# real-stanford/semantic-abstraction

Hardware: AMD Instinct MI355X
Metric: scenes/sec (relevancy+3D-UNet infer), 480x480x16-label x128^3 (higher is better)
Workload: dtype f16 (MFMA operands, fp32 accumulate; UNet hi/lo-split = fp32-equivalent); 1 GPU; end-to-end relevancy->fusion->OVSSC per scene: 480x480 RGB-D, 16 labels, ViT-B/16, 'ours' saliency config (2448 tile forwards), 128^3 voxels, 80000 input points; scene-sharded; arch=ViT-B/16, unet_precision=exact, tile_chunk_streams=1, scenes_per_gpu=26, parallelism=scene-shard x1, mode=throughput

## Files before the change

### semantic-abstraction_amd/csrc/unet.hip

```cpp
#include "semabs_common.h"

__device__ __forceinline__ int xcd_remap(int vb, int nb) {
    const int q = nb >> 3, r = nb & 7, x = vb & 7, k = vb >> 3;
    return (x < r ? x * (q + 1) : r * (q + 1) + (x - r) * q) + k;
}
__device__ __forceinline__ int xcd_persistent_tile(int vb, int G, int it, int total) {
    if (G & 7) { const long t = (long)it * G + vb; return t < total ? (int)t : -1; }
    const int x = vb & 7, j = vb >> 3, g8 = G >> 3;
    const int q = total >> 3, r = total & 7;
    const int lo = x < r ? x * (q + 1) : r * (q + 1) + (x - r) * q, cnt = q + (x < r ? 1 : 0);
    const long o = (long)it * g8 + j;
    return o < cnt ? lo + (int)o : -1;
}


template <int HID, int COUT>
__global__ __launch_bounds__(256, 2) void k_point_mlp(const float* __restrict__ xyz, const float* __restrict__ feat,
                                                   const float* __restrict__ w1, const float* __restrict__ b1,
                                                   const float* __restrict__ w2, const float* __restrict__ b2,
                                                   const float* __restrict__ w3, const float* __restrict__ b3,
                                                   float* __restrict__ out, int P, long N) {
    extern __shared__ __attribute__((aligned(16))) char smem[];
    float* sw2 = reinterpret_cast<float*>(smem);
    float* sw3 = sw2 + HID * HID;
// ... 374 lines not shown
    SEMABS_REQUIRE(sums && gamma && beta && scale && shift && C % G == 0 && nvox > 0, "semabs_gn_finalize: bad args");
    hipLaunchKernelGGL(k_gn_finalize, dim3(semabs_cdiv((long)B * C, 256)), dim3(256), 0, (hipStream_t)stream, sums, gamma, beta, scale,
                       shift, B, C, G, (double)nvox * (C / G), eps);
    SEMABS_CHECK_LAUNCH();
    return SEMABS_OK;
}

#ifdef SEMABS_TUNING
#define CONV16_ABL(c) (c)
#else
#define CONV16_ABL(c) false
#endif
struct ConvArgs {
    const void* x; void* y; const f16* w_hi; const f16* w_lo;
    const float* gn_scale; const float* gn_shift; const float* bias; const void* resid;
    int B, I0, I1, I2;
    int O0, O1, O2;
    int M0, M1, M2;
    int os, op0, op1, op2;
    int Cin, Cout, Kp;
    int ntaps; int relu;
    int is;
    int ksplit;
    signed char td0[28], td1[28], td2[28];
    double* stats;
    int ablate;
    long long* trace;
    const f16* wp_hi; const f16* wp_lo;
    int ncls; long cls_off[8];
    const float* gnb_coef = nullptr; const float* gnb_mean = nullptr; const float* gnb_rstd = nullptr; int gnb_G = 0, gnb_relu = 0;
    unsigned int* gnb_bits = nullptr;
    const unsigned int* occ = nullptr;
    const float* gnb_add = nullptr;
};

template <bool F32>
__device__ __forceinline__ void load8(const void* base, long idx, float (&v)[8]) {
    if (F32) {
        const float4* p = reinterpret_cast<const float4*>(reinterpret_cast<const float*>(base) + idx);
        float4 a = p[0], b = p[1];
        v[0] = a.x; v[1] = a.y; v[2] = a.z; v[3] = a.w; v[4] = b.x; v[5] = b.y; v[6] = b.z; v[7] = b.w;
    } else {
        f16x8 h = *reinterpret_cast<const f16x8*>(reinterpret_cast<const f16*>(base) + idx);
#pragma unroll
        for (int j = 0; j < 8; ++j) v[j] = (float)h[j];
    }
}

template <int NW, bool F32, bool CIN16, bool LDSW = false, bool CLS = false>
__global__ __launch_bounds__(256) void k_conv(ConvArgs a) {
    const int ccls = CLS ? (int)blockIdx.z : 0;
    const int cp0 = CLS ? ccls >> 2 : 0, cp1 = CLS ? (ccls >> 1) & 1 : 0, cp2 = CLS ? ccls & 1 : 0;
    const int k_ntaps = CLS ? (cp0 + 1) * (cp1 + 1) * (cp2 + 1) : a.ntaps;
    const int k_Kp = CLS ? k_ntaps * a.Cin : a.Kp;
    const int k_op0 = CLS ? cp0 : a.op0, k_op1 = CLS ? cp1 : a.op1, k_op2 = CLS ? cp2 : a.op2;
    const long k_woff = CLS ? a.cls_off[ccls] : 0;
    const f16* const k_w_hi = a.w_hi + k_woff; const f16* const k_w_lo = a.w_lo ? a.w_lo + k_woff : nullptr;
    const f16* const k_wp_hi = a.wp_hi ? a.wp_hi + k_woff : nullptr; const f16* const k_wp_lo = a.wp_lo ? a.wp_lo + k_woff : nullptr;
    constexpr int MW = 2;
    static_assert(!LDSW || (NW == 4 && !CIN16), "LDSW: four waves x four output-channel tiles");
    __shared__ __attribute__((aligned(16))) f16x8 s_w[LDSW ? 2 : 1][LDSW ? 4 : 1][2][LDSW ? 64 : 1];
    const int lane = threadIdx.x & 63, wid = threadIdx.x >> 6;
    const int vl = lane & 15, kg = lane >> 4;
    const long Mtot = (long)a.B * a.M0 * a.M1 * a.M2;
    const long mbase = ((long)blockIdx.x * 4 + wid) * (MW * 16);
    if (!LDSW && mbase >= Mtot) return;
// ... 456 lines not shown
                for (int j = 0; j < 4; ++j) st[j] += (double)ps[j];
            }
        }
    };

    auto lds_barrier = [&]() { asm volatile("s_waitcnt lgkmcnt(0)\n\ts_barrier" ::: "memory"); };
    auto brick_of = [&](int it) { return xcd_persistent_tile((int)blockIdx.x, (int)gridDim.x, it, total); };
    if (producer) {
        int it = 0, brick = brick_of(0);
        if (brick >= 0) produce(brick, 0);
        lds_barrier();
        int buf = 0;
        for (; brick >= 0; buf ^= 1) {
            const int next = brick_of(++it);
            if (next >= 0 && !CONV16_ABL(a.ablate == 2 || a.ablate >= 4)) produce(next, buf ^ 1);
            lds_barrier();
            brick = next;
        }
    } else {
        load_weights();
        lds_barrier();
        int buf = 0, it = 0;
        for (int brick = brick_of(0); brick >= 0; brick = brick_of(++it), buf ^= 1) {
            if (!CONV16_ABL(a.ablate == 1)) consume(brick, buf);
            lds_barrier();
        }
        if (a.stats) flush_stats();
        if (GNB && a.gnb_bits) conv_absmax_commit(a.gnb_bits, amax);
    }
}

#define SEMABS_CONV_GENERIC 256
#define SEMABS_CONV_PACKED 512
#ifdef SEMABS_TUNING
static int g_conv16_ablate = 0;
static long long* g_conv_trace = nullptr;
static int g_brick_persist = 0;
static int g_convt_no_line = 0;
extern "C" int semabs_conv_tune(int key, long long value) {
    if (key == 0) g_conv16_ablate = (int)value & 7;
    else if (key == 1) g_conv_trace = reinterpret_cast<long long*>(value);
    else if (key == 2) g_brick_persist = (int)value;
    else if (key == 3) g_convt_no_line = (int)value;
    return SEMABS_OK;
}
#endif

static int conv16_lds_launch(const ConvArgs& a_in, int f32, hipStream_t s) {
    ConvArgs a = a_in;
#ifdef SEMABS_TUNING
    a.ablate = g_conv16_ablate;
#endif
    if (f32) {
        constexpr int T0 = 4;
        const size_t lds = (size_t)(((T0 + 2) * C16_H1 * C16_H2 * 8 + 127) / 128 * 128) * 2 * 2 * 2 * 2;
        const long total = (long)a.B * (a.I0 / T0) * (a.I1 / C16_T1) * (a.I2 / C16_T2);
        long nb = semabs_stream_cus(s); if (nb > total) nb = total;
        if (a.gnb_coef) {
            static SemabsLdsAttr attrg;
            semabs_ensure_lds(&k_conv16_lds<true, T0, true>, (int)(lds + 32 * 192), attrg);
            hipLaunchKernelGGL((k_conv16_lds<true, T0, true>), dim3((unsigned)nb), dim3(512), lds + (size_t)a.B * 192, s, a);
            SEMABS_CHECK_LAUNCH();
            return SEMABS_OK;
        }
        if (a.occ) {
            static SemabsLdsAttr attrs;
            semabs_ensure_lds(&k_conv16_lds<true, T0, false, true>, (int)lds, attrs);
            hipLaunchKernelGGL((k_conv16_lds<true, T0, false, true>), dim3((unsigned)nb), dim3(512), lds, s, a);
            SEMABS_CHECK_LAUNCH();
            return SEMABS_OK;
        }
        static SemabsLdsAttr attr;
        semabs_ensure_lds(&k_conv16_lds<true, T0>, (int)lds, attr);
        hipLaunchKernelGGL((k_conv16_lds<true, T0>), dim3((unsigned)nb), dim3(512), lds, s, a);
    } else {
        constexpr int T0 = 8;
// ... 349 lines not shown
    }
    BRICK_STAMP(7);
}

template <bool F32, int CW, int NB, bool ONE, bool PERSIST, int TX = 16, bool GNB = false>
static int conv_brick_launch_p(const ConvArgs& a, hipStream_t s) {
    const size_t lds = (size_t)((6 * C16_H1 * (TX + 2) * 8 + 127) / 128 * 128) * (CW / 8) * 2 * (F32 ? 2 : 1);
    static int per_cu = 0;
    if (!per_cu) {
        (void)hipFuncSetAttribute(reinterpret_cast<const void*>(&k_conv_brick<F32, CW, NB, ONE, PERSIST, TX, GNB>), hipFuncAttributeMaxDynamicSharedMemorySize, (int)lds);
        int n = 0;
        if (hipOccupancyMaxActiveBlocksPerMultiprocessor(&n, k_conv_brick<F32, CW, NB, ONE, PERSIST, TX, GNB>, 512, lds) != hipSuccess || n < 1) n = 1;
        per_cu = n;
    }
    const long total = (long)(a.I0 / 4) * (a.I1 / C16_T1) * (a.I2 / TX) * a.B * (a.Cout / (NB * 16));
    SEMABS_REQUIRE(total < (1L << 30), "conv brick: too many tiles");
    long nwg = total;
    if (PERSIST) { nwg = (long)semabs_stream_cus(s) * per_cu; if (nwg > total) nwg = total; }
    ConvArgs at = a;
#ifdef SEMABS_TUNING
    at.trace = g_conv_trace;
#endif
    hipLaunchKernelGGL((k_conv_brick<F32, CW, NB, ONE, PERSIST, TX, GNB>), dim3((unsigned)nwg), dim3(512), lds, s, at, (int)total);
    SEMABS_CHECK_LAUNCH();
    return SEMABS_OK;
}
template <bool F32, int CW, int NB, bool ONE>
static int conv_brick_launch_t(const ConvArgs& a, hipStream_t s) {
#ifdef SEMABS_TUNING
    if (g_brick_persist) return conv_brick_launch_p<F32, CW, NB, ONE, true>(a, s);
#endif
    return conv_brick_launch_p<F32, CW, NB, ONE, false>(a, s);
}
static int conv_brick_launch(const ConvArgs& a, int f32, hipStream_t s) {
    if (a.gnb_coef) {
        if (a.Cin == 32) return conv_brick_launch_p<true, 32, 2, true, false, 16, true>(a, s);
        return conv_brick_launch_p<true, 32, 2, false, false, 16, true>(a, s);
    }
    if (a.I2 % C16_T2 != 0) {
        return f32 ? conv_brick_launch_p<true, 32, 2, false, false, 8>(a, s) : conv_brick_launch_p<false, 32, 2, false, false, 8>(a, s);
    }
    const long bricks = (long)a.B * (a.I0 / 4) * (a.I1 / C16_T1) * (a.I2 / C16_T2);
    if (a.Cout == 16) {
        if (a.Cin == 32) return f32 ? conv_brick_launch_t<true, 32, 1, true>(a, s) : conv_brick_launch_t<false, 32, 1, true>(a, s);
        return f32 ? conv_brick_launch_t<true, 32, 1, false>(a, s) : conv_brick_launch_t<false, 32, 1, false>(a, s);
    }
    const bool nb4 = a.Cout % 64 == 0 && bricks * (a.Cout / 64) >= 512;
    if (a.Cin == 16) {
        if (nb4) return f32 ? conv_brick_launch_t<true, 16, 4, true>(a, s) : conv_brick_launch_t<false, 16, 4, true>(a, s);
        return f32 ? conv_brick_launch_t<true, 16, 2, true>(a, s) : conv_brick_launch_t<false, 16, 2, true>(a, s);
    }
    if (a.Cin == 32) {
        if (nb4) return f32 ? conv_brick_launch_t<true, 32, 4, true>(a, s) : conv_brick_launch_t<false, 32, 4, true>(a, s);
        return f32 ? conv_brick_launch_t<true, 32, 2, true>(a, s) : conv_brick_launch_t<false, 32, 2, true>(a, s);
    }
    if (nb4) return f32 ? conv_brick_launch_t<true, 32, 4, false>(a, s) : conv_brick_launch_t<false, 32, 4, false>(a, s);
    return f32 ? conv_brick_launch_t<true, 32, 2, false>(a, s) : conv_brick_launch_t<false, 32, 2, false>(a, s);
}

__global__ void k_conv_finish(float* __restrict__ y, const float* __restrict__ bias, const float* __restrict__ resid, long n4, int C, int relu) {
    const long i = (long)blockIdx.x * blockDim.x + threadIdx.x;
    if (i >= n4) return;
    float4 v = *reinterpret_cast<float4*>(y + i * 4);
    if (bias) { const float4 b = *reinterpret_cast<const float4*>(bias + (i * 4) % C); v.x += b.x; v.y += b.y; v.z += b.z; v.w += b.w; }
    if (resid) { const float4 r = *reinterpret_cast<const float4*>(resid + i * 4); v.x += r.x; v.y += r.y; v.z += r.z; v.w += r.w; }
    if (relu == 1) { v.x = fmaxf(v.x, 0.f); v.y = fmaxf(v.y, 0.f); v.z = fmaxf(v.z, 0.f); v.w = fmaxf(v.w, 0.f); }
    else if (relu == 2) { v.x = v.x > 0.f ? v.x : 0.01f * v.x; v.y = v.y > 0.f ? v.y : 0.01f * v.y; v.z = v.z > 0.f ? v.z : 0.01f * v.z; v.w = v.w > 0.f ? v.w : 0.01f * v.w; }
    *reinterpret_cast<float4*>(y + i * 4) = v;
}

static int conv_launch(const ConvArgs& a_in, int f32, hipStream_t s) {
    ConvArgs a = a_in;
    const long Mtot = (long)a.B * a.M0 * a.M1 * a.M2;
    a.ksplit = 1;
    if (f32 && a.os == 1 && a.Cout % 64 == 0 && a.Cin % 32 == 0 && a.ntaps == 27 && Mtot <= 16384) {
        const long slices = semabs_cdiv(Mtot, 4 * 32) * (a.Cout / 64);
        int ks = (int)(2048 / (slices > 0 ? slices : 1));
        if (ks > 27) ks = 27;
        if (ks >= 3) {
// ... 5 lines not shown
            hipLaunchKernelGGL(k_conv_finish, dim3(semabs_cdiv(n4, 256)), dim3(256), 0, s, reinterpret_cast<float*>(a.y), a.bias,
                               reinterpret_cast<const float*>(a.resid), n4, a.Cout, a.relu);
            SEMABS_CHECK_LAUNCH();
            return SEMABS_OK;
        }
    }
    const int ncls = a.ncls > 0 ? a.ncls : 1;
    int nw = a.Cout >= 64 ? 4 : (a.Cout >= 32 ? 2 : 1);
    while (nw > 1 && (long)semabs_cdiv(Mtot, 4 * 32) * (a.Cout / (nw * 16)) * ncls < 1024) nw >>= 1;
    dim3 grid(semabs_cdiv(Mtot, 4 * 32), a.Cout / (nw * 16), ncls), block(256);
    const bool c16 = a.Cin == 16;
    if (a.ncls > 0) {
#define CONVC_GO(NW_, F_) hipLaunchKernelGGL((k_conv<NW_, F_, false, false, true>), grid, block, 0, s, a)
        if (f32) { if (nw == 4) CONVC_GO(4, true); else if (nw == 2) CONVC_GO(2, true); else CONVC_GO(1, true); }
        else { if (nw == 4) CONVC_GO(4, false); else if (nw == 2) CONVC_GO(2, false); else CONVC_GO(1, false); }
#undef CONVC_GO
        SEMABS_CHECK_LAUNCH();
        return SEMABS_OK;
    }
#define CONV_GO(NW_, F_, C_) hipLaunchKernelGGL((k_conv<NW_, F_, C_>), grid, block, 0, s, a)
#define CONV_NW(F_, C_) { if (nw == 4) CONV_GO(4, F_, C_); else if (nw == 2) CONV_GO(2, F_, C_); else CONV_GO(1, F_, C_); }
    if (nw == 4 && !c16) {
        if (f32) hipLaunchKernelGGL((k_conv<4, true, false, true>), grid, block, 0, s, a);
        else hipLaunchKernelGGL((k_conv<4, false, false, true>), grid, block, 0, s, a);
    }
    else if (f32) { if (c16) CONV_NW(true, true) else CONV_NW(true, false) }
    else { if (c16) CONV_NW(false, true) else CONV_NW(false, false) }
#undef CONV_NW
#undef CONV_GO
    SEMABS_CHECK_LAUNCH();
    return SEMABS_OK;
}

static int conv_common_checks(const void* x, const void* w_hi, const void* w_lo, void* y, int Cin, int Cout, int f32) {
    SEMABS_REQUIRE(x && w_hi && y, "semabs conv: null pointer");
    SEMABS_REQUIRE(!f32 || w_lo, "semabs conv: exact (fp32) mode needs the lo half of the split weights");
    SEMABS_REQUIRE(Cin == 16 || Cin % 32 == 0, "semabs conv: Cin must be 16 or a multiple of 32");
    SEMABS_REQUIRE(Cout % 16 == 0 && (Cout < 64 || Cout % 64 == 0), "semabs conv: Cout must be 16, 32 or a multiple of 64");
    return SEMABS_OK;
}

static int conv3d_impl(const void* x, const void* w_hi, const void* w_lo, void* y, const float* gn_scale, const float* gn_shift,
                       const float* bias, const void* resid, int B, int D0, int D1, int D2, int Cin, int Cout, int ksize,
                       int relu, int act_flags, double* out_sums, int out_groups, void* stream, const unsigned int* occ = nullptr) {
    if (B == 0) return SEMABS_OK;
    const int act_f32 = act_flags & 1;
    const bool bricks = !(act_flags & SEMABS_CONV_GENERIC);
    int rc = conv_common_checks(x, w_hi, w_lo, y, Cin, Cout, act_f32);
    if (rc) return rc;
    SEMABS_REQUIRE(ksize == 1 || ksize == 3, "semabs_conv3d: kernel size must be 1 or 3");
    SEMABS_REQUIRE((gn_scale == nullptr) == (gn_shift == nullptr), "semabs_conv3d: gn_scale and gn_shift go together");
    ConvArgs a;
    a.x = x; a.y = y; a.w_hi = (const f16*)w_hi; a.w_lo = (const f16*)w_lo; a.gn_scale = gn_scale; a.gn_shift = gn_shift;
    a.bias = bias; a.resid = resid; a.B = B; a.I0 = D0; a.I1 = D1; a.I2 = D2; a.O0 = D0; a.O1 = D1; a.O2 = D2;
    a.M0 = D0; a.M1 = D1; a.M2 = D2; a.os = 1; a.is = 1; a.op0 = a.op1 = a.op2 = 0; a.Cin = Cin; a.Cout = Cout; a.relu = relu;
    a.ntaps = ksize * ksize * ksize;
    a.Kp = ((a.ntaps * Cin + 31) / 32) * 32;
    a.stats = nullptr; a.ablate = 0; a.trace = nullptr; a.wp_hi = nullptr; a.wp_lo = nullptr; a.ncls = 0;
    if (act_flags & SEMABS_CONV_PACKED) {
        a.wp_hi = a.w_hi + (long)Cout * a.Kp;
        if (w_lo) a.wp_lo = a.w_lo + (long)Cout * a.Kp;
    }
    int t = 0;
    for (int kd = 0; kd < ksize; ++kd)
        for (int kh = 0; kh < ksize; ++kh)
            for (int kw = 0; kw < ksize; ++kw, ++t) { a.td0[t] = kd - ksize / 2; a.td1[t] = kh - ksize / 2; a.td2[t] = kw - ksize / 2; }
    SEMABS_REQUIRE(relu == 0 || relu == 1 || (relu == 2 && ksize == 1), "semabs_conv3d: relu must be 0, 1, or 2 (LeakyReLU, ksize 1 only)");
    SEMABS_REQUIRE(!out_sums || (out_groups > 0 && Cout % out_groups == 0), "semabs_conv3d_stats: Cout must be a multiple of out_groups");
    bool fused = false;
    if (bricks && ksize == 3 && Cin == 16 && Cout == 16 && D0 % 8 == 0 && D1 % C16_T1 == 0 && D2 % C16_T2 == 0 && (long)D0 * D1 * D2 * 16 < (1L << 31)) {
        if (out_sums && out_groups == 8) { a.stats = out_sums; fused = true; }
        a.occ = occ;
        rc = conv16_lds_launch(a, act_f32, (hipStream_t)stream);
    } else if (occ) {
        semabs_set_error("semabs_conv3d_sparse_stats: the occupancy bitmap is read by the 16 -> 16 level-0 kernel only (D0 % 8, D1 % 8, D2 % 16 == 0)");
        return SEMABS_EINVAL;
    } else if (bricks && ksize == 3 && (Cout % 32 == 0 || (Cout == 16 && Cin % 32 == 0 && D2 % C16_T2 == 0)) && (Cin == 16 || Cin % 32 == 0) && relu != 2 &&
               D0 % 4 == 0 && D1 % C16_T1 == 0 && (D2 % C16_T2 == 0 || (D2 % 8 == 0 && Cin % 32 == 0))) {
        if (out_sums && out_groups == 8 && Cout >= 32) { a.stats = out_sums; fused = true; }
        rc = conv_brick_launch(a, act_f32, (hipStream_t)stream);
    } else {
        rc = conv_launch(a, act_f32, (hipStream_t)stream);
    }
    if (rc == SEMABS_OK && out_sums && !fused) rc = semabs_gn_stats(y, out_sums, B, (long)D0 * D1 * D2, Cout, out_groups, act_f32, stream);
    return rc;
}
extern "C" int semabs_conv3d(const void* x, const void* w_hi, const void* w_lo, void* y, const float* gn_scale, const float* gn_shift,
                             const float* bias, const void* resid, int B, int D0, int D1, int D2, int Cin, int Cout, int ksize,
                             int relu, int act_f32, void* stream) {
    return conv3d_impl(x, w_hi, w_lo, y, gn_scale, gn_shift, bias, resid, B, D0, D1, D2, Cin, Cout, ksize, relu, act_f32, nullptr, 0, stream);
}
extern "C" int semabs_conv3d_stats(const void* x, const void* w_hi, const void* w_lo, void* y, const float* gn_scale, const float* gn_shift,
                                   const float* bias, const void* resid, int B, int D0, int D1, int D2, int Cin, int Cout, int ksize,
                                   int relu, int act_f32, double* out_sums, int out_groups, void* stream) {
    SEMABS_REQUIRE(out_sums, "semabs_conv3d_stats: out_sums is null");
    return conv3d_impl(x, w_hi, w_lo, y, gn_scale, gn_shift, bias, resid, B, D0, D1, D2, Cin, Cout, ksize, relu, act_f32, out_sums, out_groups, stream);
}

extern "C" int semabs_conv3d_sparse_stats(const void* x, const unsigned int* occ, const void* w_hi, const void* w_lo, void* y, const float* gn_scale, const float* gn_shift,
                                          const float* bias, const void* resid, int B, int D0, int D1, int D2, int Cin, int Cout, int ksize,
                                          int relu, int act_f32, double* out_sums, int out_groups, void* stream) {
    SEMABS_REQUIRE(out_sums && occ, "semabs_conv3d_sparse_stats: out_sums / occ is null");
    SEMABS_REQUIRE(!(act_f32 & SEMABS_CONV_GENERIC), "semabs_conv3d_sparse_stats: the generic kernel reads the whole volume");
    return conv3d_impl(x, w_hi, w_lo, y, gn_scale, gn_shift, bias, resid, B, D0, D1, D2, Cin, Cout, ksize, relu, act_f32, out_sums, out_groups, stream, occ);
}

static int conv3d_gnbwd_route(int B, int D0, int D1, int D2, int Cin, int Cout, int G, bool have_add) {
    if (B <= 0 || G <= 0) return 0;
    if (B <= 32 && Cin == 16 && Cout == 16 && D0 % 8 == 0 && D1 % C16_T1 == 0 && D2 % C16_T2 == 0 && (long)D0 * D1 * D2 * 16 < (1L << 31) && 16 % G == 0) return 1;
    if (!have_add && Cin % 32 == 0 && Cout % 32 == 0 && Cout % G == 0 && (Cout / G) % 4 == 0 && D0 % 4 == 0 && D1 % C16_T1 == 0 && D2 % C16_T2 == 0) return 2;
    return 0;
// ... 625 lines not shown
```

### semantic-abstraction_amd/train.py

```python
from __future__ import annotations

import ctypes as C
import os
from typing import Dict, List, Optional

import numpy as np
import torch

from . import _lib
from .net import VirtualGrid
from .optim import Lamb
from .unet3d import (_Conv, _ConvT, _Rec, conv_bwd_layout, conv_fwd_layout, convT_class_layout, gn_conv, linear_layout,
                     number_of_features_per_level, unet_forward)
from .weights import unet_layer_plan

RELATIONS = ["in", "behind", "in front of", "on the left of", "on the right of", "on", "[pad]"]
SLOPE = 0.01


def _taps(vals) -> bytes:
    return np.asarray(vals, np.int8).tobytes()


TAPS_CONV3 = _taps([(a - 1, b - 1, c - 1) for a in range(3) for b in range(3) for c in range(3)])
TAPS_ONE = _taps([(0, 0, 0)])


class _WeightLayouts:

    def __init__(self, dev):
        self.dev = dev
        self.maps: Dict[str, tuple] = {}
        self.src_ptr: Dict[str, int] = {}
        self.fresh: set = set()
        self._table = None

    def invalidate(self):
        self.fresh.clear()

    def refresh_all(self):
        if not self.maps or os.environ.get("SEMABS_BATCH_GATHER", "1") != "1":
            return
        keys = tuple(self.maps)
        if self._table is None or self._table[3] != keys or any(self._table[4][k] != self.src_ptr[k] for k in keys):
            rows, blk = [], 0
# ... 160 lines not shown
        sc, sh, s2 = self._scale(dZ, B, cout)
        inv = s2[1:]
        dW = self.g[key + "conv.weight"]
        scr = self._wg_scratch() if self.wgrad_tr else (None, 0)
        red = self.arena.zeros((B, cin, 2), torch.float64)
        have_red = False
        if self.mfma_wgrad and self.wgrad_tr and self.wgrad_gn and self._supported("semabs_wgrad_conv3_gn_supported", B, D0, D1, D2, cout, cin, int(scr[1])):
            _lib.call("semabs_wgrad_conv3_gn", _lib.ptr(dZ), _lib.ptr(r.x), _lib.ptr(r.mean), _lib.ptr(r.rstd), G, _lib.ptr(self.p[key + "groupnorm.weight"]),
                      _lib.ptr(self.p[key + "groupnorm.bias"]), _lib.ptr(self.p[key + "conv.weight"]), _lib.ptr(s2), _lib.ptr(dW), _lib.ptr(red),
                      B, D0, D1, D2, cout, cin, *scr, st)
            have_red = True
        elif self.mfma_wgrad and self._supported("semabs_wgrad_conv3_supported", D0, D1, D2, cout, cin, int(scr[1])):
            _lib.call("semabs_wgrad_conv3", _lib.ptr(dZ), _lib.ptr(r.x), _lib.ptr(r.scale), _lib.ptr(r.shift), _lib.ptr(s2), _lib.ptr(dW),
                      B, D0, D1, D2, cout, cin, 1, *scr, st)
        elif cin % 16 == 0 and self.mfma_wgrad:
            _lib.call("semabs_wgrad_mfma", _lib.ptr(dZ), _lib.ptr(r.x), _lib.ptr(r.scale), _lib.ptr(r.shift), _lib.ptr(s2), None, _lib.ptr(dW),
                      B, D0, D1, D2, D0, D1, D2, 1, cout, cin, 27, TAPS_CONV3, 1, *self._wg_scratch(), st)
        else:
            _lib.call("semabs_wgrad", _lib.ptr(dZ), _lib.ptr(r.x), _lib.ptr(r.scale), _lib.ptr(r.shift), _lib.ptr(dW), B, D0, D1, D2, D0, D1, D2, 1,
                      cout, cin, 27, TAPS_CONV3, 1, st)
        if have_red and self.fuse_gn_apply and self._supported("semabs_conv3d_gnbwd_supported", B, D0, D1, D2, cout, cin, G, int(add1 is not None)):
            coef = torch.empty(B, cin, 3, dtype=torch.float32, device=self.dev)
            _lib.call("semabs_gn_bwd_coef", _lib.ptr(red), _lib.ptr(self.p[key + "groupnorm.weight"]), _lib.ptr(r.rstd), _lib.ptr(inv), _lib.ptr(coef),
                      _lib.ptr(self.g[key + "groupnorm.weight"]), _lib.ptr(self.g[key + "groupnorm.bias"]), B, cin, G, nvox, st)
            dX = torch.empty(B, D0, D1, D2, cin, dtype=torch.float32, device=self.dev)
            bits = self.arena.zeros((1,), torch.int32)
            _lib.call("semabs_conv3d_gnbwd", _lib.ptr(dZ), _lib.ptr(m.bwd[0]), _lib.ptr(m.bwd[1]), _lib.ptr(dX), _lib.ptr(sc), _lib.ptr(sh), _lib.ptr(r.x),
                      _lib.ptr(r.mean), _lib.ptr(r.rstd), _lib.ptr(coef), G, _lib.ptr(add1), 1 if relu_in else 0, _lib.ptr(bits), B, D0, D1, D2, cout, cin,
                      1 | m.bwd[2], st)
            dX._semabs_absmax = bits
            return dX
        dXn = torch.empty(B, D0, D1, D2, cin, dtype=torch.float32, device=self.dev)
        _lib.call("semabs_conv3d", _lib.ptr(dZ), _lib.ptr(m.bwd[0]), _lib.ptr(m.bwd[1]), _lib.ptr(dXn), _lib.ptr(sc), _lib.ptr(sh), None, None,
                  B, D0, D1, D2, cout, cin, 3, 0, 1 | m.bwd[2], st)
        if not have_red:
            _lib.call("semabs_chan_reduce", _lib.ptr(dXn), _lib.ptr(r.x), _lib.ptr(r.mean), _lib.ptr(r.rstd), _lib.ptr(red), B, nvox, cin, G, st)
        coef = torch.empty(B, cin, 3, dtype=torch.float32, device=self.dev)
        _lib.call("semabs_gn_bwd_coef", _lib.ptr(red), _lib.ptr(self.p[key + "groupnorm.weight"]), _lib.ptr(r.rstd), _lib.ptr(inv), _lib.ptr(coef),
                  _lib.ptr(self.g[key + "groupnorm.weight"]), _lib.ptr(self.g[key + "groupnorm.bias"]), B, cin, G, nvox, st)
        dX = torch.empty_like(dXn)
        bits = self.arena.zeros((1,), torch.int32)
        _lib.call("semabs_gn_bwd_apply", _lib.ptr(dXn), _lib.ptr(r.x), _lib.ptr(r.mean), _lib.ptr(r.rstd), _lib.ptr(coef), _lib.ptr(add1), None,
                  _lib.ptr(r.x if relu_in else None), _lib.ptr(bits), _lib.ptr(dX), B, nvox, cin, G, st)
        dX._semabs_absmax = bits
        return dX

    def _block_bwd(self, recs, dOut, in_scale=None):
        r1, r2, r3 = recs
        if getattr(dOut, "_semabs_relu_masked", False) and in_scale is None:
            dS = dOut
        else:
            dS = self._ew(dOut, r3.y, 0, want_max=True, in_scale=in_scale)
        dz2 = self._conv_bwd(r3, dS, relu_in=True)
        dz1 = self._conv_bwd(r2, dz2, add1=dS, relu_in=True)
        return self._conv_bwd(r1, dz1)

    def _up_bwd(self, pre: str, xin: torch.Tensor, g: torch.Tensor):
        m = self.convs[pre]
        key = self.prefix + pre
        st = _lib.stream()
        B, D0, D1, D2, cin = xin.shape
        cout = m.cout
        self._colsum(g.view(-1, cout), self.g[key + "bias"])
        sc, sh, s2 = self._scale(g, B, cout)
        if cout % 16 == 0 and self.mfma_wgrad:
            _lib.call("semabs_wgrad_mfma", _lib.ptr(xin), _lib.ptr(g), None, None, None, _lib.ptr(s2), _lib.ptr(self.g[key + "weight"]),
                      B, D0, D1, D2, 2 * D0, 2 * D1, 2 * D2, 2, cin, cout, 27, TAPS_CONV3, 1, *self._wg_scratch(), st)
# ... 420 lines not shown
```

### semantic-abstraction_amd/unet3d.py

```python
from __future__ import annotations

import ctypes as C
from typing import Dict, List

import numpy as np
import torch

from . import _lib


def number_of_features_per_level(init_channel_number, num_levels):
    return [init_channel_number * 2 ** k for k in range(num_levels)]



def _pack_fragments(w: torch.Tensor) -> torch.Tensor:
    cout, kp = int(w.shape[0]), int(w.shape[1])
    assert cout % 16 == 0 and kp % 32 == 0
    return w.reshape(cout // 16, 16, kp // 32, 4, 8).permute(2, 0, 3, 1, 4).contiguous().reshape(-1)


def matrix_layout(m: torch.Tensor):
    rows, k = int(m.shape[0]), int(m.shape[1])
    kp = (k + 31) // 32 * 32
    if kp != k:
        m = torch.cat([m, m.new_zeros(rows, kp - k)], dim=1)
    m = m.contiguous()
    if rows % 16 == 0:
        return torch.cat([m.reshape(-1), _pack_fragments(m)]), 512
    return m.reshape(-1), 0


def conv_fwd_layout(w: torch.Tensor):
    return matrix_layout(w.permute(0, 2, 3, 4, 1).reshape(w.shape[0], -1))


def conv_bwd_layout(w: torch.Tensor):
    return matrix_layout(w.flip(2, 3, 4).permute(1, 2, 3, 4, 0).reshape(w.shape[1], -1))


def linear_layout(w: torch.Tensor, transposed: bool = False):
    return matrix_layout(w.t() if transposed else w)


def convT_class_layout(w: torch.Tensor):
    cin, cout = int(w.shape[0]), int(w.shape[1])
    mats, offs, off = [], [], 0
    for cls in range(8):
        p = (cls >> 2, (cls >> 1) & 1, cls & 1)
        cols = []
        for t0 in range(p[0] + 1):
            for t1 in range(p[1] + 1):
                for t2 in range(p[2] + 1):
                    k = [1 if pp == 0 else (0 if t == 0 else 2) for pp, t in zip(p, (t0, t1, t2))]
                    cols.append(w[:, :, k[0], k[1], k[2]].t())
        mats.append(torch.cat(cols, dim=1).contiguous())
        offs.append(off)
        off += mats[-1].numel()
    packed = cout % 16 == 0 and cin % 32 == 0
    return torch.cat([m.reshape(-1) for m in mats] + ([_pack_fragments(m) for m in mats] if packed else [])), 512 if packed else 0, offs


def _split16(w: torch.Tensor, dev):
    hi = w.to(torch.float16)
    lo = (w - hi.float()).to(torch.float16)
    return hi.to(dev).contiguous(), lo.to(dev).contiguous()


class _Conv:
    name = None
    bwd = None

    def __init__(self, weight: torch.Tensor, gn_w, gn_b, bias, groups: int, dev):
        flat, packed = conv_fwd_layout(weight.float())
        f = lambda t: None if t is None else t.float().to(dev).contiguous()
        self._set((*_split16(flat, dev), packed), weight.shape, f(gn_w), f(gn_b), f(bias), groups)

    def _set(self, fwd, wshape, gn_w, gn_b, bias, groups):
        self.w_hi, self.w_lo, self.packed = fwd
        self.cout, self.cin, self.k = int(wshape[0]), int(wshape[1]), int(wshape[2])
        self.gn_w, self.gn_b, self.bias = gn_w, gn_b, bias
        self.groups = groups if self.cin >= groups else 1

    @classmethod
    def of(cls, name, fwd, bwd, wshape, gn_w, gn_b, bias, groups):
        r = cls.__new__(cls)
        r.name, r.bwd = name, bwd
        r._set(fwd, wshape, gn_w, gn_b, bias, groups)
        return r


class _ConvT:
    name = None
    bwd = None

    def __init__(self, weight: torch.Tensor, bias, dev):
        flat, packed, offs = convT_class_layout(weight.float())
        self._set((*_split16(flat, dev), packed, offs), weight.shape, bias.float().to(dev).contiguous())

    def _set(self, fwd, wshape, bias):
        self.w_hi, self.w_lo, self.packed, offs = fwd
        self.class_off = (C.c_long * 8)(*offs)
        self.cin, self.cout = int(wshape[0]), int(wshape[1])
        self.bias = bias

    @classmethod
    def of(cls, name, fwd, bwd, wshape, bias):
        r = cls.__new__(cls)
        r.name, r.bwd = name, bwd
        r._set(fwd, wshape, bias)
        return r


class _Rec:
    __slots__ = ("name", "x", "y", "mean", "rstd", "scale", "shift")



def gn_conv(x, conv: _Conv, relu, zeros, f32, resid=None, gn=True, in_sums=None, out_groups=0, generic=False, occ=None, rec: _Rec | None = None):
    B, D0, D1, D2, Cc = x.shape
    nvox, dev, st = D0 * D1 * D2, x.device, _lib.stream()
    scale = shift = None
    if gn:
        G, sums = conv.groups, in_sums
        if sums is None:
            sums = zeros((B, G, 2), torch.float64)
            _lib.call("semabs_gn_stats", _lib.ptr(x), _lib.ptr(sums), B, nvox, Cc, G, f32, st)
        scale = torch.empty(B, Cc, dtype=torch.float32, device=dev)
        shift = torch.empty_like(scale)
        _lib.call("semabs_gn_finalize", _lib.ptr(sums), _lib.ptr(conv.gn_w), _lib.ptr(conv.gn_b), _lib.ptr(scale), _lib.ptr(shift),
                  B, Cc, G, nvox, 1e-5, st)
        if rec is not None:
            rec.mean = torch.empty(B, G, dtype=torch.float32, device=dev)
            rec.rstd = torch.empty_like(rec.mean)
            _lib.call("semabs_gn_meanrstd", _lib.ptr(sums), _lib.ptr(rec.mean), _lib.ptr(rec.rstd), B, G, nvox * (Cc // G), 1e-5, st)
    y = torch.empty(B, D0, D1, D2, conv.cout, dtype=torch.float32 if f32 else torch.float16, device=dev)
    if rec is not None:
        rec.name, rec.x, rec.y, rec.scale, rec.shift = conv.name, x, y, scale, shift
    args = (_lib.ptr(x), _lib.ptr(conv.w_hi), _lib.ptr(conv.w_lo), _lib.ptr(y), _lib.ptr(scale), _lib.ptr(shift),
            _lib.ptr(conv.bias), _lib.ptr(resid), B, D0, D1, D2, conv.cin, conv.cout, conv.k, int(relu), f32 | (256 if generic else 0) | conv.packed)
    if not out_groups:
        assert occ is None
        _lib.call("semabs_conv3d", *args, st)
        return y, None
    out_sums = zeros((B, out_groups, 2), torch.float64)
    if occ is not None:
        _lib.call("semabs_conv3d_sparse_stats", args[0], _lib.ptr(occ), *args[1:], _lib.ptr(out_sums), out_groups, st)
    else:
        _lib.call("semabs_conv3d_stats", *args, _lib.ptr(out_sums), out_groups, st)
    return y, out_sums


def res_block(x, convs, zeros, f32, in_sums=None, occ=None, tape=None):
    r1, r2, r3 = (None,) * 3 if tape is None else (_Rec(), _Rec(), _Rec())
    out1, s1 = gn_conv(x, convs[0], True, zeros, f32, in_sums=in_sums, out_groups=convs[1].groups, occ=occ, rec=r1)
    out2, s2 = gn_conv(out1, convs[1], True, zeros, f32, in_sums=s1, out_groups=convs[2].groups, rec=r2)
    y, _ = gn_conv(out2, convs[2], True, zeros, f32, resid=out1, in_sums=s2, rec=r3)
    if tape is not None:
        tape.append(("block", r1, r2, r3))
    return y


def maxpool(x, f32):
    B, D0, D1, D2, Cc = x.shape
    y = torch.empty(B, D0 // 2, D1 // 2, D2 // 2, Cc, dtype=x.dtype, device=x.device)
    _lib.call("semabs_maxpool3d", _lib.ptr(x), _lib.ptr(y), B, D0, D1, D2, Cc, f32, _lib.stream())
    return y


def up_conv(x, skip, ct: _ConvT, zeros, f32, out_groups=0, generic=False):
    B, D0, D1, D2, _ = x.shape
    assert tuple(skip.shape) == (B, 2 * D0, 2 * D1, 2 * D2, ct.cout)
    y = torch.empty_like(skip)
# ... 151 lines not shown
```

Before: 8.691 scenes/s.

## Add producer/consumer warp-specialized brick conv kernel with unit-packed weights

```diff
diff --git a/semantic-abstraction_amd/csrc/unet.hip b/semantic-abstraction_amd/csrc/unet.hip
--- a/semantic-abstraction_amd/csrc/unet.hip
+++ b/semantic-abstraction_amd/csrc/unet.hip
@@ -430,6 +430,7 @@
     unsigned int* gnb_bits = nullptr;
     const unsigned int* occ = nullptr;
     const float* gnb_add = nullptr;
+    const f16* wu_hi = nullptr; const f16* wu_lo = nullptr;
 };
 
 template <bool F32>
@@ -952,16 +953,19 @@
 
 #define SEMABS_CONV_GENERIC 256
 #define SEMABS_CONV_PACKED 512
+#define SEMABS_CONV_UNITS 1024
 #ifdef SEMABS_TUNING
 static int g_conv16_ablate = 0;
 static long long* g_conv_trace = nullptr;
 static int g_brick_persist = 0;
+static int g_brick_pc = 0;
 static int g_convt_no_line = 0;
 extern "C" int semabs_conv_tune(int key, long long value) {
     if (key == 0) g_conv16_ablate = (int)value & 7;
     else if (key == 1) g_conv_trace = reinterpret_cast<long long*>(value);
     else if (key == 2) g_brick_persist = (int)value;
     else if (key == 3) g_convt_no_line = (int)value;
+    else if (key == 4) g_brick_pc = (int)value;
     return SEMABS_OK;
 }
 #endif
@@ -1377,6 +1381,315 @@
 #endif
     return conv_brick_launch_p<F32, CW, NB, ONE, false>(a, s);
 }
+static constexpr int pc_toff(int t) { return (((t / 9) * C16_H1 + (t / 3) % 3) * C16_H2 + t % 3) * 8; }
+template <bool F32, int NB>
+__global__ __launch_bounds__(512) void k_conv_brick_pc(ConvArgs a, int total) {
+    constexpr int T0 = 4, H0 = T0 + 2, HX = C16_H2, HALO = H0 * C16_H1 * HX, R = 8, NSTEPS = 14;
+    constexpr int PLANE = (HALO * 8 + 127) / 128 * 128;
+    constexpr int BUF_EL = PLANE * 2 * (F32 ? 2 : 1);
+    extern __shared__ __attribute__((aligned(16))) char smem[];
+    const int tid = threadIdx.x, lane = tid & 63;
+    const int wid = __builtin_amdgcn_readfirstlane(tid >> 6);
+    const int n2 = a.I2 / C16_T2, n1 = a.I1 / C16_T1;
+    const int per_vol = (a.I0 / T0) * n1 * n2;
+    const int Cin = a.Cin, nun = Cin >> 4;
+    auto decode = [&](int t, int& b, int& cout0, int& z0, int& y0, int& x0) {
+        int br = t % per_vol; t /= per_vol;
+        b = t % a.B; cout0 = (t / a.B) * (NB * 16);
+        const int t2 = br % n2; br /= n2;
+        z0 = (br / n1) * T0; y0 = (br % n1) * C16_T1; x0 = t2 * C16_T2;
+    };
+    auto tile_of = [&](int it) { return xcd_persistent_tile((int)blockIdx.x, (int)gridDim.x, it, total); };
+    auto lds_barrier = [&]() { asm volatile("s_waitcnt lgkmcnt(0)\n\ts_barrier" ::: "memory"); };
+
+    if (wid >= 4) {
+        const int ptid = tid - 256;
+        const int hsel = (ptid >> 3) & 1;
+        const int vsub = (ptid & 7) + ((ptid >> 4) << 3);
+        constexpr int NT = (HALO + 127) / 128;
+        const bool has_gn = a.gn_scale != nullptr;
+        float gs[8], gh[8];
+        unsigned inb = 0;
+        [[maybe_unused]] float4 ra[NT], rb[NT];
+        [[maybe_unused]] f16x8 rh[NT];
+        auto issue = [&](int tile, int u) {
+            int b, cout0, z0, y0, x0;
+            decode(tile, b, cout0, z0, y0, x0);
+            const int ch = u * 16 + hsel * 8;
+            if (has_gn) {
+                const float4* ps = reinterpret_cast<const float4*>(a.gn_scale + (long)b * Cin + ch);
+                const float4* pt = reinterpret_cast<const float4*>(a.gn_shift + (long)b * Cin + ch);
+                const float4 s0 = ps[0], s1 = ps[1], h0 = pt[0], h1 = pt[1];
+                gs[0] = s0.x; gs[1] = s0.y; gs[2] = s0.z; gs[3] = s0.w; gs[4] = s1.x; gs[5] = s1.y; gs[6] = s1.z; gs[7] = s1.w;
+                gh[0] = h0.x; gh[1] = h0.y; gh[2] = h0.z; gh[3] = h0.w; gh[4] = h1.x; gh[5] = h1.y; gh[6] = h1.z; gh[7] = h1.w;
+            } else {
+#pragma unroll
+                for (int j = 0; j < 8; ++j) { gs[j] = 1.f; gh[j] = 0.f; }
+            }
+            const size_t vbase = (size_t)b * a.I0 * a.I1 * a.I2 * Cin + ch;
+            const float* xb = reinterpret_cast<const float*>(a.x) + vbase;
+            const f16* xbh = reinterpret_cast<const f16*>(a.x) + vbase;
+            inb = 0;
+#pragma unroll
+            for (int k = 0; k < NT; ++k) {
+                const int v = min(vsub + k * 128, HALO - 1);
+                const int hx = v % HX, hy = (v / HX) % C16_H1, hz = v / (HX * C16_H1);
+                const int gz = z0 + hz - 1, gy = y0 + hy - 1, gx = x0 + hx - 1;
+                if (gz >= 0 && gz < a.I0 && gy >= 0 && gy < a.I1 && gx >= 0 && gx < a.I2) inb |= 1u << k;
+                const int cz = min(max(gz, 0), a.I0 - 1), cy = min(max(gy, 0), a.I1 - 1), cx = min(max(gx, 0), a.I2 - 1);
+                const unsigned eo = (unsigned)((cz * a.I1 + cy) * a.I2 + cx) * (unsigned)Cin;
+                if constexpr (F32) { ra[k] = *reinterpret_cast<const float4*>(xb + eo); rb[k] = *reinterpret_cast<const float4*>(xb + eo + 4); }
+                else rh[k] = *reinterpret_cast<const f16x8*>(xbh + eo);
+            }
+        };
+        auto commit = [&](int buf) {
+            f16* s_hi = reinterpret_cast<f16*>(smem) + buf * BUF_EL + hsel * PLANE;
+            f16* s_lo = s_hi + PLANE * 2;
+#pragma unroll
+            for (int k = 0; k < NT; ++k) {
+                const int v = vsub + k * 128;
+                const bool in = (inb >> k) & 1u;
+                float raw[8];
+                if constexpr (F32) { raw[0] = ra[k].x; raw[1] = ra[k].y; raw[2] = ra[k].z; raw[3] = ra[k].w; raw[4] = rb[k].x; raw[5] = rb[k].y; raw[6] = rb[k].z; raw[7] = rb[k].w; }
+                else {
+#pragma unroll
+                    for (int c = 0; c < 8; ++c) raw[c] = (float)rh[k][c];
+                }
+                f16x8 h, l;
+#pragma unroll
+                for (int c = 0; c < 8; ++c) {
+                    const float val = in ? raw[c] * gs[c] + gh[c] : 0.f;
+                    h[c] = (f16)val;
+                    if (F32) l[c] = (f16)(val - (float)h[c]);
+                }
+                if (v < HALO) {
+                    *reinterpret_cast<f16x8*>(s_hi + v * 8) = h;
+                    if (F32) *reinterpret_cast<f16x8*>(s_lo + v * 8) = l;
+                }
+            }
+        };
+        int it = 0, pt = tile_of(0), pu = 0;
+        auto advance = [&]() { if (++pu == nun) { pu = 0; pt = tile_of(++it); } };
+        bool cur = pt >= 0;
+        if (cur) { issue(pt, 0); commit(0); advance(); if (pt >= 0) issue(pt, pu); }
+        lds_barrier();
+        for (int g = 0; cur; ++g) {
+            const bool nxt = pt >= 0;
+            if (nxt) {
+                commit((g + 1) & 1);
+                advance();
+                if (pt >= 0) issue(pt, pu);
+            }
+            lds_barrier();
+            cur = nxt;
+        }
+        lds_barrier();
+    } else {
+        const int vl = lane & 15, kg = lane >> 4, half = kg & 1, tsel = kg >> 1;
+        const int ncb = a.Cout >> 4;
+        const bool units = Cin == 16 ? a.wp_hi != nullptr : a.wu_hi != nullptr;
+        const f16* const wsrc_h = units ? (Cin == 16 ? a.wp_hi : a.wu_hi) : a.w_hi;
+        const f16* const wsrc_l = units ? (Cin == 16 ? a.wp_lo : a.wu_lo) : a.w_lo;
+        const long u_stride = units ? (long)NSTEPS * ncb * 512 : 16;
+        const long s_stride = units ? (long)ncb * 512 : 2L * Cin;
+        const long nb_stride = units ? 512 : 16L * a.Kp;
+        const bool zero_dead = !units && Cin > 16 && tsel;
+        auto w_lane = [&](int cout0) -> long {
+            return units ? (long)(cout0 >> 4) * 512 + lane * 8 : (long)(cout0 + vl) * a.Kp + (long)tsel * Cin + half * 8;
+        };
+        f16x8 wA_h[NB], wA_l[NB], wB_h[NB], wB_l[NB];
+        auto load_w = [&](long off, bool last, f16x8* wh, f16x8* wl) {
+            if (last && zero_dead) off -= Cin;
+#pragma unroll
+            for (int nb = 0; nb < NB; ++nb) {
+                wh[nb] = *reinterpret_cast<const f16x8*>(wsrc_h + off + nb * nb_stride);
+                if (F32) wl[nb] = *reinterpret_cast<const f16x8*>(wsrc_l + off + nb * nb_stride);
+                if (last) {
+#pragma unroll
+                    for (int e = 0; e < 8; ++e) { wh[nb][e] = zero_dead ? (f16)0.f : wh[nb][e]; if (F32) wl[nb][e] = zero_dead ? (f16)0.f : wl[nb][e]; }
+                }
+            }
+        };
+        const int fbase = half * PLANE + (wid * C16_H1 * HX + vl) * 8;
+        f32x4 acc[R][NB];
+        auto kloop = [&](int buf, long woff, long wnext) {
+            const f16* s_hi = reinterpret_cast<const f16*>(smem) + buf * BUF_EL + fbase;
+            const f16* s_lo = s_hi + PLANE * 2;
+            f16x8 xh[R], xl[R];
+            {
+                const int off = tsel ? pc_toff(1) : pc_toff(0);
+#pragma unroll
+                for (int r = 0; r < R; ++r) {
+                    xh[r] = *reinterpret_cast<const f16x8*>(s_hi + off + r * (HX * 8));
+                    if (F32) xl[r] = *reinterpret_cast<const f16x8*>(s_lo + off + r * (HX * 8));
+                }
+            }
+#pragma unroll
+            for (int s = 0; s < NSTEPS; ++s) {
+                f16x8* wh = (s & 1) ? wB_h : wA_h; f16x8* wl = (s & 1) ? wB_l : wA_l;
+                f16x8* whn = (s & 1) ? wA_h : wB_h; f16x8* wln = (s & 1) ? wA_l : wB_l;
+                const bool more = s + 1 < NSTEPS;
+                load_w(more ? woff + (s + 1) * s_stride : wnext, s + 1 == NSTEPS - 1, whn, wln);
+                const int tb = 2 * (s + 1) + 1 < 27 ? 2 * (s + 1) + 1 : 26;
+                const int offn = more ? (tsel ? pc_toff(tb) : pc_toff(2 * (s + 1))) : 0;
+                __builtin_amdgcn_sched_barrier(0);
+#pragma unroll
+                for (int nb = 0; nb < NB; ++nb) {
+                    const bool lastb = nb == NB - 1;
+#pragma unroll
+                    for (int r = 0; r < R; ++r) {
+                        acc[r][nb] = __builtin_amdgcn_mfma_f32_16x16x32_f16(wh[nb], xh[r], acc[r][nb], 0, 0, 0);
+                        if (!F32 && lastb && more) { xh[r] = *reinterpret_cast<const f16x8*>(s_hi + offn + r * (HX * 8)); __builtin_amdgcn_sched_barrier(0); }
+                    }
+                    if (F32) {
+#pragma unroll
+                        for (int r = 0; r < R; ++r) {
+                            acc[r][nb] = __builtin_amdgcn_mfma_f32_16x16x32_f16(wl[nb], xh[r], acc[r][nb], 0, 0, 0);
+                            if (lastb && more) { xh[r] = *reinterpret_cast<const f16x8*>(s_hi + offn + r * (HX * 8)); __builtin_amdgcn_sched_barrier(0); }
+                        }
+#pragma unroll
+                        for (int r = 0; r < R; ++r) {
+                            acc[r][nb] = __builtin_amdgcn_mfma_f32_16x16x32_f16(wh[nb], xl[r], acc[r][nb], 0, 0, 0);
+                            if (lastb && more) { xl[r] = *reinterpret_cast<const f16x8*>(s_lo + offn + r * (HX * 8)); __builtin_amdgcn_sched_barrier(0); }
+                        }
+                    }
+                }
+                __builtin_amdgcn_sched_barrier(0);
+            }
+        };
+        const int v2 = lane >> 2, k2 = lane & 3;
+        const int src = (k2 * 16 + v2) << 2;
+        const int cg = a.Cout >> 3;
+        constexpr int NSLOT = NB * 8;
+        float* const s_stat = reinterpret_cast<float*>(smem + (size_t)BUF_EL * 2 * 2);
+        if (a.stats && wid == 0 && lane < 2 * NSLOT) s_stat[lane] = 0.f;
+        double run = 0.0;
+        int st_b = -1, st_c0 = 0;
+        int pend_p = -1, pend_b = 0, pend_c0 = 0;
+        auto flush_stats = [&]() {
+            if (st_b >= 0 && lane < NSLOT) atomicAdd(a.stats + ((long)st_b * 8 + (st_c0 + (lane >> 3) * 16 + 4 * ((lane >> 1) & 3)) / cg) * 2 + (lane & 1), run);
+            run = 0.0;
+        };
+        auto collect_stats = [&]() {
+            if (pend_p >= 0 && wid == 0) {
+                if (pend_b != st_b || pend_c0 != st_c0) { flush_stats(); st_b = pend_b; st_c0 = pend_c0; }
+                if (lane < NSLOT) { float* s = s_stat + pend_p * NSLOT + lane; run += (double)*s; *s = 0.f; }
+            }
+            pend_p = -1;
+        };
+        int tpar = 0;
+        auto epilogue = [&](int b, int cout0, int z0, int y0, int x0) {
+            const size_t vol = (size_t)b * a.I0 * a.I1 * a.I2 * a.Cout;
+            unsigned obase[R];
+            float q[R][NB][4];
+#pragma unroll
+            for (int r = 0; r < R; ++r) {
+                obase[r] = (unsigned)(((z0 + wid) * a.I1 + (y0 + r)) * a.I2 + (x0 + v2)) * (unsigned)a.Cout + (unsigned)(cout0 + 4 * k2);
+#pragma unroll
+                for (int nb = 0; nb < NB; ++nb) {
+                    const size_t oi = vol + obase[r] + nb * 16;
+                    if (a.resid) {
+                        if (F32) { const float4 t = *reinterpret_cast<const float4*>(reinterpret_cast<const float*>(a.resid) + oi); q[r][nb][0] = t.x; q[r][nb][1] = t.y; q[r][nb][2] = t.z; q[r][nb][3] = t.w; }
+                        else { const f16x4 t = *reinterpret_cast<const f16x4*>(reinterpret_cast<const f16*>(a.resid) + oi); q[r][nb][0] = (float)t[0]; q[r][nb][1] = (float)t[1]; q[r][nb][2] = (float)t[2]; q[r][nb][3] = (float)t[3]; }
+                    } else {
+                        q[r][nb][0] = q[r][nb][1] = q[r][nb][2] = q[r][nb][3] = 0.f;
+                    }
+                }
+            }
+            float4 bv[NB];
+#pragma unroll
+            for (int nb = 0; nb < NB; ++nb) bv[nb] = a.bias ? *reinterpret_cast<const float4*>(a.bias + cout0 + nb * 16 + 4 * k2) : make_float4(0.f, 0.f, 0.f, 0.f);
+            const float relu_floor = a.relu ? 0.f : -__builtin_inff();
+            float st_s[NB], st_q[NB];
+#pragma unroll
+            for (int nb = 0; nb < NB; ++nb) { st_s[nb] = 0.f; st_q[nb] = 0.f; }
+            __builtin_amdgcn_sched_barrier(0);
+#pragma unroll
+            for (int r = 0; r < R; ++r) {
+#pragma unroll
+                for (int nb = 0; nb < NB; ++nb) {
+                    const size_t oi = vol + obase[r] + nb * 16;
+                    const float a0 = acc[r][nb][0], a1 = acc[r][nb][1], a2 = acc[r][nb][2], a3 = acc[r][nb][3];
+                    float o[4];
+                    o[0] = __int_as_float(__builtin_amdgcn_ds_bpermute(src, __float_as_int(a0)));
+                    o[1] = __int_as_float(__builtin_amdgcn_ds_bpermute(src, __float_as_int(a1)));
+                    o[2] = __int_as_float(__builtin_amdgcn_ds_bpermute(src, __float_as_int(a2)));
+                    o[3] = __int_as_float(__builtin_amdgcn_ds_bpermute(src, __float_as_int(a3)));
+                    o[0] = fmaxf(o[0] + q[r][nb][0] + bv[nb].x, relu_floor); o[1] = fmaxf(o[1] + q[r][nb][1] + bv[nb].y, relu_floor);
+                    o[2] = fmaxf(o[2] + q[r][nb][2] + bv[nb].z, relu_floor); o[3] = fmaxf(o[3] + q[r][nb][3] + bv[nb].w, relu_floor);
+                    if (F32) *reinterpret_cast<float4*>(reinterpret_cast<float*>(a.y) + oi) = make_float4(o[0], o[1], o[2], o[3]);
+                    else {
+                        f16x4 h; h[0] = (f16)o[0]; h[1] = (f16)o[1]; h[2] = (f16)o[2]; h[3] = (f16)o[3]; *reinterpret_cast<f16x4*>(reinterpret_cast<f16*>(a.y) + oi) = h;
+#pragma unroll
+                        for (int e = 0; e < 4; ++e) o[e] = (float)h[e];
+                    }
+                    st_s[nb] += (o[0] + o[1]) + (o[2] + o[3]);
+                    st_q[nb] += (o[0] * o[0] + o[1] * o[1]) + (o[2] * o[2] + o[3] * o[3]);
+                }
+            }
+            if (a.stats) {
+#pragma unroll
+                for (int nb = 0; nb < NB; ++nb) {
+                    float vs = st_s[nb], vq = st_q[nb];
+#pragma unroll
+                    for (int m = 4; m < 64; m <<= 1) { vs += __shfl_xor(vs, m, 64); vq += __shfl_xor(vq, m, 64); }
+                    if (v2 == 0) { atomicAdd(&s_stat[tpar * NSLOT + (nb * 4 + k2) * 2], vs); atomicAdd(&s_stat[tpar * NSLOT + (nb * 4 + k2) * 2 + 1], vq); }
+                }
+                pend_p = tpar; pend_b = b; pend_c0 = cout0;
+            }
+            tpar ^= 1;
+        };
+
+        int it = 0, tile = tile_of(0);
+        long woff = 0;
+        if (tile >= 0) {
+            int b, cout0, z0, y0, x0;
+            decode(tile, b, cout0, z0, y0, x0);
+            woff = w_lane(cout0);
+            load_w(woff, false, wA_h, wA_l);
+        }
+        lds_barrier();
+        int g = 0;
+        while (tile >= 0) {
+            int b, cout0, z0, y0, x0;
+            decode(tile, b, cout0, z0, y0, x0);
+            const int ntile = tile_of(++it);
+            long wtile = woff;
+            if (ntile >= 0) { int nb_, nc0, nz, ny, nx; decode(ntile, nb_, nc0, nz, ny, nx); wtile = w_lane(nc0); }
+#pragma unroll
+            for (int r = 0; r < R; ++r)
+#pragma unroll
+                for (int nb = 0; nb < NB; ++nb) acc[r][nb] = f32x4{0.f, 0.f, 0.f, 0.f};
+#pragma unroll 1
+            for (int u = 0; u < nun; ++u, ++g) {
+                const long wnext = u + 1 < nun ? woff + u_stride : wtile;
+                kloop(g & 1, woff, wnext);
+                lds_barrier();
+                if (u == 0) collect_stats();
+                woff = wnext;
+            }
+            epilogue(b, cout0, z0, y0, x0);
+            tile = ntile;
+        }
+        lds_barrier();
+        collect_stats();
+        if (a.stats && wid == 0) flush_stats();
+    }
+}
+
+template <bool F32, int NB>
+static int conv_brick_pc_launch(const ConvArgs& a, hipStream_t s) {
+    const size_t lds = (size_t)((6 * C16_H1 * C16_H2 * 8 + 127) / 128 * 128) * 2 * (F32 ? 2 : 1) * 2 * 2 + 2 * NB * 8 * sizeof(float);
+    static SemabsLdsAttr attr;
+    semabs_ensure_lds(&k_conv_brick_pc<F32, NB>, (int)lds, attr);
+    const long total = (long)(a.I0 / 4) * (a.I1 / C16_T1) * (a.I2 / C16_T2) * a.B * (a.Cout / (NB * 16));
+    SEMABS_REQUIRE(total < (1L << 30), "conv brick: too many tiles");
+    long nwg = semabs_stream_cus(s); if (nwg > total) nwg = total;
+    hipLaunchKernelGGL((k_conv_brick_pc<F32, NB>), dim3((unsigned)nwg), dim3(512), lds, s, a, (int)total);
+    SEMABS_CHECK_LAUNCH();
+    return SEMABS_OK;
+}
+
 static int conv_brick_launch(const ConvArgs& a, int f32, hipStream_t s) {
     if (a.gnb_coef) {
         if (a.Cin == 32) return conv_brick_launch_p<true, 32, 2, true, false, 16, true>(a, s);
@@ -1385,11 +1698,18 @@
     if (a.I2 % C16_T2 != 0) {
         return f32 ? conv_brick_launch_p<true, 32, 2, false, false, 8>(a, s) : conv_brick_launch_p<false, 32, 2, false, false, 8>(a, s);
     }
-    const long bricks = (long)a.B * (a.I0 / 4) * (a.I1 / C16_T1) * (a.I2 / C16_T2);
     if (a.Cout == 16) {
         if (a.Cin == 32) return f32 ? conv_brick_launch_t<true, 32, 1, true>(a, s) : conv_brick_launch_t<false, 32, 1, true>(a, s);
         return f32 ? conv_brick_launch_t<true, 32, 1, false>(a, s) : conv_brick_launch_t<false, 32, 1, false>(a, s);
     }
+    const bool fits = (long)a.I0 * a.I1 * a.I2 * (a.Cin > a.Cout ? a.Cin : a.Cout) < (1L << 31);
+    bool pc = a.Cin % 32 != 0 ? a.Cin != 16 : (fits && ((a.Cin >= 64 && a.Cout >= 128) || (f32 && a.Cin == 32 && a.Cout == 32)));
+#ifdef SEMABS_TUNING
+    if (g_brick_pc == 1) pc = a.Cin % 32 != 0 && a.Cin != 16;
+    else if (g_brick_pc == 2) pc = fits || (a.Cin % 32 != 0 && a.Cin != 16);
+#endif
+    if (pc) return f32 ? conv_brick_pc_launch<true, 2>(a, s) : conv_brick_pc_launch<false, 2>(a, s);
+    const long bricks = (long)a.B * (a.I0 / 4) * (a.I1 / C16_T1) * (a.I2 / C16_T2);
     const bool nb4 = a.Cout % 64 == 0 && bricks * (a.Cout / 64) >= 512;
     if (a.Cin == 16) {
         if (nb4) return f32 ? conv_brick_launch_t<true, 16, 4, true>(a, s) : conv_brick_launch_t<false, 16, 4, true>(a, s);
@@ -1461,10 +1781,10 @@
     return SEMABS_OK;
 }
 
-static int conv_common_checks(const void* x, const void* w_hi, const void* w_lo, void* y, int Cin, int Cout, int f32) {
+static int conv_common_checks(const void* x, const void* w_hi, const void* w_lo, void* y, int Cin, int Cout, int f32, bool cin16 = false) {
     SEMABS_REQUIRE(x && w_hi && y, "semabs conv: null pointer");
     SEMABS_REQUIRE(!f32 || w_lo, "semabs conv: exact (fp32) mode needs the lo half of the split weights");
-    SEMABS_REQUIRE(Cin == 16 || Cin % 32 == 0, "semabs conv: Cin must be 16 or a multiple of 32");
+    SEMABS_REQUIRE(Cin == 16 || Cin % 32 == 0 || (cin16 && Cin % 16 == 0), "semabs conv: Cin must be 16 or a multiple of 32 (any multiple of 16 on the brick kernel's shapes)");
     SEMABS_REQUIRE(Cout % 16 == 0 && (Cout < 64 || Cout % 64 == 0), "semabs conv: Cout must be 16, 32 or a multiple of 64");
     return SEMABS_OK;
 }
@@ -1475,7 +1795,9 @@
     if (B == 0) return SEMABS_OK;
     const int act_f32 = act_flags & 1;
     const bool bricks = !(act_flags & SEMABS_CONV_GENERIC);
-    int rc = conv_common_checks(x, w_hi, w_lo, y, Cin, Cout, act_f32);
+    const bool pc = bricks && ksize == 3 && !occ && Cin % 16 == 0 && Cout % 32 == 0 && relu != 2 && D0 % 4 == 0 && D1 % C16_T1 == 0 && D2 % C16_T2 == 0 &&
+                    (long)D0 * D1 * D2 * (Cin > Cout ? Cin : Cout) < (1L << 31);
+    int rc = conv_common_checks(x, w_hi, w_lo, y, Cin, Cout, act_f32, pc);
     if (rc) return rc;
     SEMABS_REQUIRE(ksize == 1 || ksize == 3, "semabs_conv3d: kernel size must be 1 or 3");
     SEMABS_REQUIRE((gn_scale == nullptr) == (gn_shift == nullptr), "semabs_conv3d: gn_scale and gn_shift go together");
@@ -1489,6 +1811,10 @@
     if (act_flags & SEMABS_CONV_PACKED) {
         a.wp_hi = a.w_hi + (long)Cout * a.Kp;
         if (w_lo) a.wp_lo = a.w_lo + (long)Cout * a.Kp;
+    }
+    if (pc && Cin > 16 && (act_flags & SEMABS_CONV_UNITS)) {
+        a.wu_hi = a.w_hi + 2L * Cout * a.Kp;
+        if (w_lo) a.wu_lo = a.w_lo + 2L * Cout * a.Kp;
     }
     int t = 0;
     for (int kd = 0; kd < ksize; ++kd)
@@ -1504,8 +1830,8 @@
     } else if (occ) {
         semabs_set_error("semabs_conv3d_sparse_stats: the occupancy bitmap is read by the 16 -> 16 level-0 kernel only (D0 % 8, D1 % 8, D2 % 16 == 0)");
         return SEMABS_EINVAL;
-    } else if (bricks && ksize == 3 && (Cout % 32 == 0 || (Cout == 16 && Cin % 32 == 0 && D2 % C16_T2 == 0)) && (Cin == 16 || Cin % 32 == 0) && relu != 2 &&
-               D0 % 4 == 0 && D1 % C16_T1 == 0 && (D2 % C16_T2 == 0 || (D2 % 8 == 0 && Cin % 32 == 0))) {
+    } else if (pc || (bricks && ksize == 3 && (Cout % 32 == 0 || (Cout == 16 && Cin % 32 == 0 && D2 % C16_T2 == 0)) && (Cin == 16 || Cin % 32 == 0) && relu != 2 &&
+               D0 % 4 == 0 && D1 % C16_T1 == 0 && (D2 % C16_T2 == 0 || (D2 % 8 == 0 && Cin % 32 == 0)))) {
         if (out_sums && out_groups == 8 && Cout >= 32) { a.stats = out_sums; fused = true; }
         rc = conv_brick_launch(a, act_f32, (hipStream_t)stream);
     } else {
diff --git a/semantic-abstraction_amd/train.py b/semantic-abstraction_amd/train.py
--- a/semantic-abstraction_amd/train.py
+++ b/semantic-abstraction_amd/train.py
@@ -10,7 +10,7 @@
 from . import _lib
 from .net import VirtualGrid
 from .optim import Lamb
-from .unet3d import (_Conv, _ConvT, _Rec, conv_bwd_layout, conv_fwd_layout, convT_class_layout, gn_conv, linear_layout,
+from .unet3d import (_Conv, _ConvT, _Rec, conv_bwd_layout, conv_fwd_layout, conv_unit_flag, convT_class_layout, gn_conv, linear_layout,
                      number_of_features_per_level, unet_forward)
 from .weights import unet_layer_plan
 
@@ -237,7 +237,7 @@
             return dX
         dXn = torch.empty(B, D0, D1, D2, cin, dtype=torch.float32, device=self.dev)
         _lib.call("semabs_conv3d", _lib.ptr(dZ), _lib.ptr(m.bwd[0]), _lib.ptr(m.bwd[1]), _lib.ptr(dXn), _lib.ptr(sc), _lib.ptr(sh), None, None,
-                  B, D0, D1, D2, cout, cin, 3, 0, 1 | m.bwd[2], st)
+                  B, D0, D1, D2, cout, cin, 3, 0, 1 | m.bwd[2] | conv_unit_flag((cin, cout, 3)), st)
         if not have_red:
             _lib.call("semabs_chan_reduce", _lib.ptr(dXn), _lib.ptr(r.x), _lib.ptr(r.mean), _lib.ptr(r.rstd), _lib.ptr(red), B, nvox, cin, G, st)
         coef = torch.empty(B, cin, 3, dtype=torch.float32, device=self.dev)
diff --git a/semantic-abstraction_amd/unet3d.py b/semantic-abstraction_amd/unet3d.py
--- a/semantic-abstraction_amd/unet3d.py
+++ b/semantic-abstraction_amd/unet3d.py
@@ -31,12 +31,31 @@
     return m.reshape(-1), 0
 
 
+def conv_unit_flag(wshape) -> int:
+    cout, cin, k = int(wshape[0]), int(wshape[1]), int(wshape[2])
+    return 1024 if k == 3 and cin > 16 and cin % 16 == 0 and cout % 32 == 0 else 0
+
+
+def _pack_units(w: torch.Tensor) -> torch.Tensor:
+    cout, cin = int(w.shape[0]), int(w.shape[2])
+    w = torch.cat([w, w.new_zeros(cout, 1, cin)], dim=1)
+    return w.reshape(cout // 16, 16, 14, 2, cin // 16, 2, 8).permute(4, 2, 0, 3, 5, 1, 6).contiguous().reshape(-1)
+
+
 def conv_fwd_layout(w: torch.Tensor):
-    return matrix_layout(w.permute(0, 2, 3, 4, 1).reshape(w.shape[0], -1))
+    m = w.permute(0, 2, 3, 4, 1)
+    flat, flag = matrix_layout(m.reshape(w.shape[0], -1))
+    if conv_unit_flag(w.shape):
+        flat = torch.cat([flat, _pack_units(m.reshape(w.shape[0], 27, w.shape[1]))])
+    return flat, flag
 
 
 def conv_bwd_layout(w: torch.Tensor):
-    return matrix_layout(w.flip(2, 3, 4).permute(1, 2, 3, 4, 0).reshape(w.shape[1], -1))
+    m = w.flip(2, 3, 4).permute(1, 2, 3, 4, 0)
+    flat, flag = matrix_layout(m.reshape(w.shape[1], -1))
+    if conv_unit_flag((w.shape[1], w.shape[0], w.shape[2])):
+        flat = torch.cat([flat, _pack_units(m.reshape(w.shape[1], 27, w.shape[0]))])
+    return flat, flag
 
 
 def linear_layout(w: torch.Tensor, transposed: bool = False):
@@ -79,6 +98,7 @@
     def _set(self, fwd, wshape, gn_w, gn_b, bias, groups):
         self.w_hi, self.w_lo, self.packed = fwd
         self.cout, self.cin, self.k = int(wshape[0]), int(wshape[1]), int(wshape[2])
+        self.units = conv_unit_flag(wshape)
         self.gn_w, self.gn_b, self.bias = gn_w, gn_b, bias
         self.groups = groups if self.cin >= groups else 1
 
@@ -138,7 +158,7 @@
     if rec is not None:
         rec.name, rec.x, rec.y, rec.scale, rec.shift = conv.name, x, y, scale, shift
     args = (_lib.ptr(x), _lib.ptr(conv.w_hi), _lib.ptr(conv.w_lo), _lib.ptr(y), _lib.ptr(scale), _lib.ptr(shift),
-            _lib.ptr(conv.bias), _lib.ptr(resid), B, D0, D1, D2, conv.cin, conv.cout, conv.k, int(relu), f32 | (256 if generic else 0) | conv.packed)
+            _lib.ptr(conv.bias), _lib.ptr(resid), B, D0, D1, D2, conv.cin, conv.cout, conv.k, int(relu), f32 | (256 if generic else 0) | conv.packed | conv.units)
     if not out_groups:
         assert occ is None
         _lib.call("semabs_conv3d", *args, st)
```

Measured after the change: 8.707 scenes/s, median of 6. No clear change (+0.2%).
